# Lagrange-Labs/mapreduce-plonky2

Hardware: AMD Instinct MI355X
Metric: leaf proofs/sec (whole node) + NTT GB/s vs HBM peak, 2^20-row table build, 1/2/4/8 GPU (higher is better)
Workload: dtype u64 (Goldilocks field)

## Files before the change

### mapreduce-plonky2_amd/csrc/poseidon.cuh

```cuda
#pragma once
#include "gl.cuh"
#include "perm_constants.h"

#pragma push_macro("MP2G_DEVCONST")
#undef MP2G_DEVCONST
#undef MP2G_PERM_CONSTANTS_H
#define MP2G_DEVCONST static constexpr
namespace p2_cx {
#include "perm_constants.h"
constexpr u64 diag_shl32(int i) { return (u64)(((unsigned __int128)POSEIDON2_DIAG_M1[i] << 32) % GL_P); }
constexpr unsigned diag_narrow(int i = 0) {
  return i == 12 ? 0u : (GL_MULC_NARROW(POSEIDON2_DIAG_M1[i], diag_shl32(i)) ? 1u << i : 0u) | diag_narrow(i + 1);
}
}
#pragma pop_macro("MP2G_DEVCONST")
MP2G_DEVCONST uint64_t POSEIDON2_DIAG_M1_SHL32[12] = {
  p2_cx::diag_shl32(0), p2_cx::diag_shl32(1), p2_cx::diag_shl32(2), p2_cx::diag_shl32(3), p2_cx::diag_shl32(4), p2_cx::diag_shl32(5),
  p2_cx::diag_shl32(6), p2_cx::diag_shl32(7), p2_cx::diag_shl32(8), p2_cx::diag_shl32(9), p2_cx::diag_shl32(10), p2_cx::diag_shl32(11),
};
constexpr unsigned POSEIDON2_DIAG_NARROW = p2_cx::diag_narrow();
static_assert(POSEIDON2_DIAG_NARROW == 0xcfeu, "limbs 0, 8 and 9 take gl_mulc_addw's carry (profiles/p2_diag measured this split)");

#define MP2G_POSEIDON2 0
#define MP2G_POSEIDON 1

#define c_p2_ext POSEIDON2_RC_EXT
#define c_p2_int POSEIDON2_RC_INT
#define c_p2_diag POSEIDON2_DIAG_M1
#define c_p2_diag_shl32 POSEIDON2_DIAG_M1_SHL32
#define c_p_rc POSEIDON_RC

GLHD u64 p2_sbox(u64 x, u64 rc) {
  u64 t = gl_addw(x, rc);
  u64 t2 = gl_mulw(t, t), t4 = gl_mulw(t2, t2), t3 = gl_mulw(t, t2);
  return gl_mulw(t3, t4);
}
GLHD void p2_m4_plain(u64& a, u64& b, u64& c, u64& d) {
  u64 t0 = a + b, t1 = c + d;
  u64 t2 = (b << 1) + t1, t3 = (d << 1) + t0;
  u64 t4 = (t1 << 2) + t3, t5 = (t0 << 2) + t2;
  a = t3 + t5; b = t5; c = t2 + t4; d = t4;
}
GLHD void p2_external_half(u64 v[12]) {
  p2_m4_plain(v[0], v[1], v[2], v[3]);
  p2_m4_plain(v[4], v[5], v[6], v[7]);
  p2_m4_plain(v[8], v[9], v[10], v[11]);
#pragma unroll
  for (int i = 0; i < 4; i++) {
    u64 sum = v[i] + v[4 + i] + v[8 + i];
    v[i] += sum; v[4 + i] += sum; v[8 + i] += sum;
  }
}
template <bool RC>
GLHD void p2_external_rc(u64 s[12], const u64* rc) {
  u64 lo[12], hi[12];
#pragma unroll
  for (int i = 0; i < 12; i++) { lo[i] = (u32)s[i]; hi[i] = s[i] >> 32; }
  p2_external_half(lo);
  p2_external_half(hi);
#if defined(__HIP_DEVICE_COMPILE__)
#pragma unroll
  for (int i = 0; i < 12; i++) {
    u64 L = lo[i], H = hi[i];
    if (RC) { L += (u64)(u32)rc[i]; H += rc[i] >> 32; }
    H += L >> 32;
    s[i] = gl_reduce96w(gl_mk((u32)L, (u32)H), H >> 32);
  }
#else
#pragma unroll
  for (int i = 0; i < 12; i++) {
    u32 c0, c1, top = (u32)(hi[i] >> 32);
    u32 l0 = (u32)lo[i];
    u32 l1 = __builtin_addc((u32)(lo[i] >> 32), (u32)hi[i], 0u, &c0);
    top += c0;
    if (RC) {
      const u64 k = rc[i];
      l0 = __builtin_addc(l0, (u32)k, 0u, &c0);
      l1 = __builtin_addc(l1, (u32)(k >> 32), c0, &c1);
      top += c1;
    }
    s[i] = gl_reduce96w(gl_mk(l0, l1), top);
  }
#endif
}
GLHD void p2_external(u64 s[12]) { p2_external_rc<false>(s, nullptr); }
GLHD u64 p2_sbox0(u64 t) {
  u64 t2 = gl_mulw_k(t, t), t4 = gl_mulw_k(t2, t2), t3 = gl_mulw_k(t, t2);
  return gl_mulw_k(t3, t4);
}
GLHD u64 p2_diag_mul_addw(int i, u64 a, u64 c) {
  if ((POSEIDON2_DIAG_NARROW >> i) & 1) return gl_mulc_addw<true>(a, c_p2_diag[i], c_p2_diag_shl32[i], c);
  return gl_mulc_addw<false>(a, c_p2_diag[i], c_p2_diag_shl32[i], c);
}
GLHD void p2_internal(u64 s[12]) {
#if defined(__HIP_DEVICE_COMPILE__)
  u64 al = 0, ah = 0;
#pragma unroll
  for (int i = 0; i < 12; i++) {
    al += (u64)(u32)s[i];
    ah += s[i] >> 32;
  }
  ah += al >> 32;
  const u64 sum = gl_reduce96w(gl_mk((u32)al, (u32)ah), ah >> 32);
#pragma unroll
  for (int i = 0; i < 12; i++) {
    s[i] = p2_diag_mul_addw(i, s[i], sum);
    __builtin_amdgcn_sched_barrier(0);
  }
#else
  u64 acc = s[0];
  u64 top = 0;
#pragma unroll
  for (int i = 1; i < 12; i++) {
    bool c = __builtin_add_overflow(acc, s[i], &acc);
    top += c ? 1 : 0;
  }
#pragma unroll
  for (int i = 0; i < 12; i++) {
    u64 lo, hi;
    gl_mul_wide(s[i], c_p2_diag[i], lo, hi);
    bool c = __builtin_add_overflow(lo, acc, &lo);
    s[i] = gl_reduce128w(lo, hi + top + (c ? 1 : 0));
  }
#endif
}
GLHD void poseidon2_perm(u64 s[12]) {
  p2_external_rc<true>(s, c_p2_ext);
#pragma unroll 1
  for (int r = 0; r < 4; r++) {
#pragma unroll
    for (int i = 0; i < 12; i++) s[i] = p2_sbox0(s[i]);
    if (r < 3) p2_external_rc<true>(s, c_p2_ext + 12 * (r + 1)); else p2_external(s);
  }
#pragma unroll 11
  for (int r = 0; r < 22; r++) {
    s[0] = p2_sbox0(gl_addw(s[0], c_p2_int[r]));
    p2_internal(s);
  }
#pragma unroll
  for (int i = 0; i < 12; i++) s[i] = gl_addw(s[i], c_p2_ext[48 + i]);
#pragma unroll 1
  for (int r = 4; r < 8; r++) {
#pragma unroll
    for (int i = 0; i < 12; i++) s[i] = p2_sbox0(s[i]);
    if (r < 7) p2_external_rc<true>(s, c_p2_ext + 12 * (r + 1)); else p2_external(s);
  }
#pragma unroll
  for (int i = 0; i < 12; i++) s[i] = gl_canon(s[i]);
}

template <bool RC>
GLHD void poseidon_mds_rc(u64 s[12], const u64* rc) {
  const u32 circ[12] = {17, 15, 41, 16, 2, 28, 13, 13, 39, 18, 34, 20};
  u64 lo[12], hi[12];
#pragma unroll
  for (int i = 0; i < 12; i++) { lo[i] = (u32)s[i]; hi[i] = s[i] >> 32; }
  u64 out[12];
#pragma unroll
  for (int r = 0; r < 12; r++) {
    u64 al = 0, ah = 0;
#pragma unroll
    for (int i = 0; i < 12; i++) {
      al += lo[(i + r) % 12] * circ[i];
      ah += hi[(i + r) % 12] * circ[i];
    }
    if (r == 0) { al += lo[0] * 8; ah += hi[0] * 8; }
    u32 c0, c1, top = (u32)(ah >> 32);
    u32 l0 = (u32)al;
    u32 l1 = __builtin_addc((u32)(al >> 32), (u32)ah, 0u, &c0);
    top += c0;
    if (RC) {
      const u64 k = rc[r];
      l0 = __builtin_addc(l0, (u32)k, 0u, &c0);
      l1 = __builtin_addc(l1, (u32)(k >> 32), c0, &c1);
      top += c1;
    }
    out[r] = gl_reduce96w(gl_mk(l0, l1), top);
  }
#pragma unroll
  for (int i = 0; i < 12; i++) s[i] = out[i];
}
GLHD void poseidon_mds(u64 s[12]) { poseidon_mds_rc<false>(s, nullptr); }
GLHD void poseidon_perm(u64 s[12]) {
#pragma unroll
  for (int i = 0; i < 12; i++) s[i] = gl_addw(s[i], c_p_rc[i]);
#pragma unroll 1
  for (int r = 0; r < 30; r++) {
    if (r < 4 || r >= 26) {
#pragma unroll
      for (int i = 0; i < 12; i++) s[i] = p2_sbox0(s[i]);
    } else {
      s[0] = p2_sbox0(s[0]);
    }
    if (r < 29) poseidon_mds_rc<true>(s, c_p_rc + 12 * (r + 1)); else poseidon_mds(s);
  }
#pragma unroll
  for (int i = 0; i < 12; i++) s[i] = gl_canon(s[i]);
}
template <int VARIANT>
GLHD void perm(u64 s[12]) {
  if (VARIANT == MP2G_POSEIDON2) poseidon2_perm(s); else poseidon_perm(s);
}
template <int VARIANT>
GLD void two_to_one(const u64 l[4], const u64 r[4], u64 out[4]) {
  u64 s[12];
#pragma unroll
  for (int i = 0; i < 4; i++) { s[i] = l[i]; s[4 + i] = r[i]; s[8 + i] = 0; }
  perm<VARIANT>(s);
#pragma unroll
  for (int i = 0; i < 4; i++) out[i] = s[i];
}
```

Baseline: 1030.

## Compute Poseidon2 external MDS in wrapping 64-bit with byte-dot-product carry recovery

```diff
diff --git a/mapreduce-plonky2_amd/csrc/poseidon.cuh b/mapreduce-plonky2_amd/csrc/poseidon.cuh
--- a/mapreduce-plonky2_amd/csrc/poseidon.cuh
+++ b/mapreduce-plonky2_amd/csrc/poseidon.cuh
@@ -52,7 +52,7 @@
   }
 }
 template <bool RC>
-GLHD void p2_external_rc(u64 s[12], const u64* rc) {
+GLHD void p2_external_rc_halves(u64 s[12], const u64* rc) {
   u64 lo[12], hi[12];
 #pragma unroll
   for (int i = 0; i < 12; i++) { lo[i] = (u32)s[i]; hi[i] = s[i] >> 32; }
@@ -83,7 +83,46 @@
   }
 #endif
 }
-GLHD void p2_external(u64 s[12]) { p2_external_rc<false>(s, nullptr); }
+constexpr int P2_EXT_SPLIT = 56;
+constexpr u64 P2_EXT_ROWSUM = 2 * (5 + 7 + 1 + 3) + (5 + 7 + 1 + 3) + (5 + 7 + 1 + 3);
+constexpr u64 P2_EXT_LOW = (1ull << P2_EXT_SPLIT) - 1;
+static_assert(P2_EXT_ROWSUM == 64 && P2_EXT_SPLIT == 56, "circ(2 M4, M4, M4); the split is a byte boundary (v_perm_b32, v_dot4_u32_u8)");
+static_assert(((P2_EXT_ROWSUM * P2_EXT_LOW + P2_EXT_LOW) >> P2_EXT_SPLIT) < 256, "the low parts carry less than 2^8 into the top bytes' sum");
+static_assert(((P2_EXT_ROWSUM * 255 + 255 + 255) >> 8) < (1u << 7), "top < 2^7");
+constexpr u32 p2_m4_bytes(int r) {
+  return r == 0 ? (5u | 7u << 8 | 1u << 16 | 3u << 24) : r == 1 ? (4u | 6u << 8 | 1u << 16 | 1u << 24)
+       : r == 2 ? (1u | 3u << 8 | 5u << 16 | 7u << 24) : (1u | 1u << 8 | 4u << 16 | 6u << 24);
+}
+template <bool RC>
+GLHD void p2_external_rc(u64 s[12], const u64* rc) {
+#if defined(__HIP_DEVICE_COMPILE__)
+  u32 tb[3];
+#pragma unroll
+  for (int b = 0; b < 3; b++) {
+    const u32 h01 = __builtin_amdgcn_perm((u32)(s[4 * b + 1] >> 32), (u32)(s[4 * b] >> 32), 0x0c0c0703u);
+    const u32 h23 = __builtin_amdgcn_perm((u32)(s[4 * b + 3] >> 32), (u32)(s[4 * b + 2] >> 32), 0x0c0c0703u);
+    tb[b] = __builtin_amdgcn_perm(h23, h01, 0x05040100u);
+  }
+  u32 g[4];
+#pragma unroll
+  for (int r = 0; r < 4; r++) {
+    g[r] = __builtin_amdgcn_udot4(tb[0], p2_m4_bytes(r), 255u, false);
+    g[r] = __builtin_amdgcn_udot4(tb[1], p2_m4_bytes(r), g[r], false);
+    g[r] = __builtin_amdgcn_udot4(tb[2], p2_m4_bytes(r), g[r], false);
+  }
+  p2_external_half(s);
+#pragma unroll
+  for (int i = 0; i < 12; i++) {
+    u64 x = s[i];
+    u32 u = __builtin_amdgcn_udot4(tb[i / 4], p2_m4_bytes(i % 4), g[i % 4], false);
+    if (RC) { x += rc[i]; u += (u32)(rc[i] >> P2_EXT_SPLIT); }
+    s[i] = gl_reduce96w(x, (u - (u32)(x >> P2_EXT_SPLIT)) >> 8);
+  }
+#else
+  p2_external_rc_halves<RC>(s, rc);
+#endif
+}
+GLHD void p2_external(u64 s[12]) { p2_external_rc_halves<false>(s, nullptr); }
 GLHD u64 p2_sbox0(u64 t) {
   u64 t2 = gl_mulw_k(t, t), t4 = gl_mulw_k(t2, t2), t3 = gl_mulw_k(t, t2);
   return gl_mulw_k(t3, t4);
@@ -130,7 +169,7 @@
   for (int r = 0; r < 4; r++) {
 #pragma unroll
     for (int i = 0; i < 12; i++) s[i] = p2_sbox0(s[i]);
-    if (r < 3) p2_external_rc<true>(s, c_p2_ext + 12 * (r + 1)); else p2_external(s);
+    if (r < 3) p2_external_rc<true>(s, c_p2_ext + 12 * (r + 1)); else p2_external_rc<false>(s, nullptr);
   }
 #pragma unroll 11
   for (int r = 0; r < 22; r++) {
@@ -143,7 +182,7 @@
   for (int r = 4; r < 8; r++) {
 #pragma unroll
     for (int i = 0; i < 12; i++) s[i] = p2_sbox0(s[i]);
-    if (r < 7) p2_external_rc<true>(s, c_p2_ext + 12 * (r + 1)); else p2_external(s);
+    if (r < 7) p2_external_rc<true>(s, c_p2_ext + 12 * (r + 1)); else p2_external_rc<false>(s, nullptr);
   }
 #pragma unroll
   for (int i = 0; i < 12; i++) s[i] = gl_canon(s[i]);
```

Result: no change. 1036 (median of 6 runs) (+0.5%).
